# ChicyChen/LOCO-Edit

Measured on AMD Instinct MI355X. Metric: edit-directions/sec (top-5 PMP-Jacobian SVD @256^2) + vT cos-sim vs ref, higher is better.
Workload: dtype bf16x3 (split-bf16 MFMA operands, fp32 accumulate + fp32 storage); 1 GPU; CelebA-HQ DDPM 256x256 top-5 local basis (l_eye-sized mask, L=2400), t=0.6T, 12 power iterations, one GPU; multi_gpu_form=single, probes_total=5, probes_per_gpu=5, kept=5, n_iter=12, mask_L=2400, weights=synthetic seed 0, streams=2

## Files before the change

loco-edit_amd/csrc/conv_bf16.hip:

```cpp
#include "kernels.h"
#include <cstdio>
#include <cstdlib>

namespace loco {

enum : int { PR_BF16X3 = 0, PR_F16 = 1 };
template <int PR, int TAPS, int MODE> void launch_tile_b(const ConvArgs& a, hipStream_t st);
template <int PR, int MODE> void launch_kcat_b(const ConvArgs& a, hipStream_t st);
template <int PR, int MODE> void launch_pair_b(const ConvArgs& a, hipStream_t st);
void launch_conv_gemm(const ConvArgs& a, hipStream_t st);
template <int PR> void launch_poly_b(const ConvArgs& a, hipStream_t st);
template <int PR> void launch_poly_in_b(const ConvArgs& a, hipStream_t st);

template <int PR>
static void launch_lowp(const ConvArgs& a, int taps, hipStream_t st) {
#ifdef LOCO_DIAG
    if (a.cot_d && (taps != 1 || a.gemm || a.nsplit > 1 || a.Cin2 > 0 || (a.Cout % conv_bf16_tile_couts(a)) != 0 || a.st_kind == ST_TAN || a.st_kind == ST_COT)) {
        fprintf(stderr, "loco: ConvArgs::cot_d on a launch whose epilogue has no norm-cotangent term (taps %d, gemm %d, nsplit %d, Cout %d, st_kind %d)\n",
                taps, a.gemm, a.nsplit, a.Cout, a.st_kind);
        abort();
    }
#endif
    if constexpr (PR == PR_BF16X3) {
        if (taps == 1 && a.gemm) { launch_conv_gemm(a, st); return; }
    }
    if (taps == 9 && a.poly == 2) { launch_poly_in_b<PR>(a, st); return; }
    if (taps == 9 && a.poly) { launch_poly_b<PR>(a, st); return; }
    if (taps == 9 && a.Cin2 > 0) {
        if (a.mode == CM_GN_SILU) launch_kcat_b<PR, CM_GN_SILU>(a, st);
        else if (a.mode == CM_GN_GELU) launch_kcat_b<PR, CM_GN_GELU>(a, st);
        else launch_kcat_b<PR, CM_TAN_SILU>(a, st);
        return;
    }
    if constexpr (PR == PR_BF16X3) {
        if (taps == 9 && a.pair) {
            switch (a.mode) {
                case CM_NONE: launch_pair_b<PR, CM_NONE>(a, st); break;
                case CM_GN_SILU: launch_pair_b<PR, CM_GN_SILU>(a, st); break;
                case CM_TAN_SILU: launch_pair_b<PR, CM_TAN_SILU>(a, st); break;
                default: launch_pair_b<PR, CM_COT_SILU>(a, st); break;
            }
            return;
        }
    }
    if (taps == 9) {
        switch (a.mode) {
            case CM_NONE: launch_tile_b<PR, 9, CM_NONE>(a, st); break;
            case CM_GN_SILU: launch_tile_b<PR, 9, CM_GN_SILU>(a, st); break;
            case CM_GN_GELU: launch_tile_b<PR, 9, CM_GN_GELU>(a, st); break;
            case CM_TAN_SILU: launch_tile_b<PR, 9, CM_TAN_SILU>(a, st); break;
            case CM_COT_SILU: launch_tile_b<PR, 9, CM_COT_SILU>(a, st); break;
            default: launch_tile_b<PR, 9, CM_GN>(a, st); break;
        }
    } else {
        switch (a.mode) {
            case CM_NONE: launch_tile_b<PR, 1, CM_NONE>(a, st); break;
            default: launch_tile_b<PR, 1, CM_GN>(a, st); break;
        }
    }
}
void launch_conv_bf16x3(const ConvArgs& a, int taps, hipStream_t st) { launch_lowp<PR_BF16X3>(a, taps, st); }
void launch_conv_f16(const ConvArgs& a, int taps, hipStream_t st) { launch_lowp<PR_F16>(a, taps, st); }

}
```

loco-edit_amd/csrc/conv_plan.hip:

```cpp
#include "kernels.h"
#include <cstdio>
#include <cstdlib>

namespace loco {

constexpr int BKC = 16;
constexpr int BKF = 8;

static const int kMT[6] = {128, 128, 32, 64, 128, 128}, kNT[6] = {128, 64, 128, 64, 256, 256};

static int env_int(const char* name, int dflt) {
    const char* e = getenv(name);
    return e ? atoi(e) : dflt;
}
static int pick_tile(int Cout, int HW) {
    if (HW >= 128) return Cout > 32 ? 0 : 2;
    return Cout > 64 ? 1 : 3;
}

static int conv_pick_nsplit(int Cin, int Cout, int Hout, int Wout, int B) {
    const int t = pick_tile(Cout, Hout * Wout);
    long blocks = (long)((Hout * Wout) / kNT[t]) * ((Cout + kMT[t] - 1) / kMT[t]) * B;
    int nchunks = (Cin + BKF - 1) / BKF;
    if (blocks >= 384 || nchunks < 8) return 1;
    int want = (int)((512 + blocks - 1) / blocks);
    int maxs = nchunks / 4;
    if (want > maxs) want = maxs;
    if (want > 32) want = 32;
    return want < 1 ? 1 : want;
}

static int conv_bf16_pick_tile(int Cout, int HW, int B, int tile_override) {
    if (B <= 1 && HW <= 1024 && HW >= 64 && (Cout % 64) == 0) return 3;
    int t = pick_tile(Cout, HW);
    if (t == 0 && HW >= 256) {
        if (tile_override >= 0) return tile_override;
        return 5;
    }
    return t;
}

constexpr int kTile0MaxHW = 65536;

static int bf16_tile_of(const ConvArgs& a, int tile_override = -1) {
    int tile = conv_bf16_pick_tile(a.Cout, a.Hout * a.Wout, a.B, tile_override);
    if (tile == 4) tile = 5;
    if (tile == 5 && a.taps == 1 && !a.gemm && a.B >= 2 && a.Hout * a.Wout <= kTile0MaxHW) return 0;
    if (a.stride == 2 && tile == 5) tile = 0;
    return tile;
}
static int tile_for(const ConvArgs& a, int prec, int tile_override) {
    return prec ? bf16_tile_of(a, tile_override) : pick_tile(a.Cout, a.Hout * a.Wout);
}
static int conv_bf16_tile_pixels(const ConvArgs& a) { return a.poly == 1 ? 512 : a.gemm ? 256 : kNT[a.tile]; }
int conv_bf16_tile_couts(const ConvArgs& a) { return a.gemm ? 64 * a.gemm_tm : kMT[a.tile]; }

static bool conv_poly_ok(const ConvEnv& e, const ConvArgs& a, int taps) {
    static const bool on = env_int("LOCO_POLYPHASE", 1) != 0;
    if (!on || e.prec < 1 || taps != 9 || a.mode != CM_NONE || !(a.upsample || a.zins) || a.stride != 1) return false;
    if (!(e.prec == 2 ? a.wph : a.wpb) || !a.in_padded || a.res || a.Cin2 > 0 || a.cot_d) return false;
    if (a.upsample ? a.pad != 1 : (a.pad != 1 && a.pad != 2)) return false;
    if ((a.Cin % BKC) != 0 || (a.Cout % 128) != 0 || a.B < 2) return false;
    if (a.Hin * a.Win < 4096 || a.Win < 32 || (a.Win % 32) != 0 || (a.Hin % 8) != 0) return false;
    return a.Hout == 2 * a.Hin && a.Wout == 2 * a.Win;
}
static bool conv_poly_in_ok(const ConvEnv& e, const ConvArgs& a, int taps) {
    static const bool on = env_int("LOCO_POLYPHASE", 1) != 0;
    if (!on || e.prec < 1 || taps != 9 || a.mode != CM_NONE || !a.pool2 || a.upsample || a.zins || a.stride != 1 || a.pad != 1) return false;
    if (!(e.prec == 2 ? a.wqh : a.wqb) || a.res || a.bias2 || a.Cin2 > 0 || a.cot_d) return false;
    if ((a.Cin % BKC) != 0 || (a.Cout % 128) != 0 || a.B < 2 || ((a.Hin | a.Win) & 1)) return false;
    if (a.Hout * a.Wout < 4096 || a.Wout < 32 || (a.Wout % 32) != 0 || (a.Hout % 8) != 0) return false;
    return a.Hin == 2 * a.Hout && a.Win == 2 * a.Wout;
}

static int conv_bf16_pick_nsplit(int Cin, int Cout, int Hout, int Wout, int B, int chip_share, int taps, int lanes) {
    const int HW = Hout * Wout;
    int t = conv_bf16_pick_tile(Cout, HW, B, -1);
    if (t == 4) t = 5;
    if (taps == 1 && t == 5 && B >= 2 && HW <= kTile0MaxHW) t = 0;
    long blocks = (long)(HW / kNT[t]) * ((Cout + kMT[t] - 1) / kMT[t]) * B;
    int nchunks = (Cin + BKC - 1) / BKC;
    int target = chip_share > 1 ? 256 / chip_share : (lanes == 2 ? 240 : 256);
    if (target < 32) target = 32;
    if (blocks >= target / 2 || nchunks < 8) return 1;
    int want = (int)(target / blocks);
    int maxs = nchunks / 4;
    if (want > maxs) want = maxs;
    if (want > 32) want = 32;
    return want < 1 ? 1 : want;
}

static bool conv_lowp_can_kcat(const ConvArgs& a) {
    static const bool on = env_int("LOCO_KCAT", 1) != 0;
    return on && a.Cin2 > 0 && a.nsplit == 1 && bf16_tile_of(a) == 5 && a.stride == 1 && !a.upsample && !a.zins && a.pad == 1 &&
           (a.Cin % BKC) == 0 && (a.Cin2 % BKC) == 0 && a.in_padded &&
           (a.mode == CM_GN_SILU || a.mode == CM_GN_GELU || a.mode == CM_TAN_SILU);
}
static bool conv_lowp_can_fuse_stats(const ConvArgs& a) {
    return a.nsplit <= 1 && !a.gemm && (a.Cout % conv_bf16_tile_couts(a)) == 0;
}

static bool conv_pair_ok(const ConvArgs& a) {
    static const bool on = env_int("LOCO_CONV_PAIR", 1) != 0;
    if (!on || a.poly || a.Hout * a.Wout < 16384 || a.taps != 9 || a.Cin2 > 0 || a.nsplit != 1 || a.stride != 1 || a.upsample || a.zins ||
        a.pad != 1 || !a.in_padded || (a.Cin % (2 * BKC)) != 0 || (a.Cout % 128) != 0 || (a.Wout % 32) != 0 || (a.Hout % 8) != 0)
        return false;
    if (!(a.mode == CM_NONE || a.mode == CM_GN_SILU || a.mode == CM_TAN_SILU || a.mode == CM_COT_SILU)) return false;
    return a.tile == 5;
}

static ConvArgs conv_shift_batch(const ConvArgs& a, int nb) {
    ConvArgs t = a;
    t.B = a.B - nb;
    t.in += (long)nb * a.in_bs; t.out += (long)nb * a.out_bs;
    if (t.prim) t.prim += (long)nb * a.prim_bs;
    if (t.bias2) t.bias2 += (long)nb * a.bias2_bs;
    if (t.res) t.res += (long)nb * a.res_bs;
    if (t.sc) { t.sc += (long)nb * a.scsh_bs; t.sh += (long)nb * a.scsh_bs; }
    if (t.mr) t.mr += (long)nb * a.mr_bs;
    if (t.tst) t.tst += (long)nb * a.tst_bs;
    if (t.tc) t.tc += (long)nb * a.tc_bs;
    if (t.in2) t.in2 += (long)nb * a.in2_bs;
    if (t.cot_d) { t.cot_d += (long)nb * a.cot_d_bs; t.cot_tc += (long)nb * a.cot_tc_bs; }
    if (t.st_part) t.st_part += (long)nb * a.Cout * ((a.Hout * a.Wout) / conv_bf16_tile_pixels(a)) * 2;
    return t;
}

static void conv_gemm_plan(ConvArgs& a) {
    static const bool on = env_int("LOCO_CONV_GEMM", 1) != 0;
    a.gemm = 0;
    const long HW = (long)a.Hout * a.Wout;
    if (!on || a.stride != 1 || a.upsample || a.zins || (a.Cin % BKC) != 0 || a.Cin < 320 || (HW % 256) != 0 || (a.Wout % 16) != 0 ||
        a.Cout < 128 || !a.partial || a.Cin2 > 0 || !(a.mode == CM_NONE || a.mode == CM_GN) || a.cot_d)
        return;
    {
        const int TW = a.Wout < 32 ? a.Wout : 32;
        if ((256 % TW) != 0 || (a.Wout % TW) != 0 || (a.Hout % (256 / TW)) != 0) return;
    }
    static const int all_shapes = env_int("LOCO_GEMM_ALL", 0);
    if (!all_shapes && !(a.Cout >= 640 && (a.Cout >= 4 * a.Cin || a.Cin >= 2560))) return;
    const int pad256 = (a.Cout + 255) / 256 * 256;
    const int tm = (pad256 * 10 <= a.Cout * 11) ? 4 : 2;
    const int mt = 64 * tm;
    const long tiles = (HW / 256) * ((a.Cout + mt - 1) / mt) * a.B;
    const size_t rec_floats = (size_t)a.B * a.Cin * HW;
    int ns = 1;
    if (tiles < 192) {
        const int nchunks = a.Cin / BKC;
        ns = (int)((256 + tiles - 1) / tiles);
        if (ns > 8) ns = 8;
        while (ns > 1 && nchunks / ns < 8) --ns;
        while (ns > 1 && (size_t)ns * a.B * a.Cout * HW + rec_floats > a.partial_floats) --ns;
    }
    if ((ns > 1 ? (size_t)ns * a.B * a.Cout * HW : 0) + rec_floats > a.partial_floats) return;
    a.gemm = 1; a.gemm_tm = tm; a.nsplit = ns;
}

void conv_plan_family(ConvArgs& a, int prec) {
    if (prec == 1 && a.taps == 1) conv_gemm_plan(a);
}

// ... 16 lines not shown
    const int nchunks = (a.Cin + 15) / 16;
    while (s > 1 && nchunks / s < 4) --s;
    const size_t one = (size_t)(r / per_probe) * a.Cout * a.Hout * a.Wout;
    while (s > 1 && (size_t)s * one > partial_floats) --s;
    *split = s;
    return s > 1 ? (int)(r / per_probe) : 0;
}

static int stats_route(const ConvEnv& e, const StatAsk* q, bool want, ConvArgs& x, int s0, int B, int* keep_ntile) {
    if (!q || q->kind == ST_NONE) return SR_NONE;
    const int alone = q->norm ? SR_ALONE : SR_NONE;
    if (!want) return alone;
    if (x.nsplit > 1) return !q->norm ? SR_NONE : ((x.Hout * x.Wout) % 4 == 0 ? SR_SPLITK : SR_ALONE);
    const int ntile = (x.Hout * x.Wout) / conv_bf16_tile_pixels(x);
    const size_t need = (size_t)x.B * x.Cout * ntile * 2;
    const int epi = q->norm ? SR_EPI : SR_KEEP;
    const bool kept = q->keep && s0 == 0 && x.B == B && need <= q->keep_floats;
    if (q->kind == ST_FWD && x.poly != 1 && conv_lowp_can_fuse_stats(x) && (kept || (q->norm && need <= e.stpart_floats))) {
        x.st_part = kept ? q->keep : e.stpart; x.st_kind = ST_FWD;
        if (kept) *keep_ntile = ntile;
        return epi;
    }
    const bool cot_cache = q->kind == ST_COT && q->norm && q->sx && x.poly != 1;
    if ((q->kind == ST_TAN || cot_cache) && e.fuse_lin && !x.cot_d && conv_lowp_can_fuse_stats(x)) {
        const size_t lane_off = (size_t)e.lane_s0 * (q->keep_floats / e.max_batch);
        const bool keptl = q->kind == ST_TAN && q->keep && s0 == 0 && x.B == B && lane_off + need <= q->keep_floats;
        if (keptl || (q->norm && need <= e.stpart_floats)) {
            x.st_part = keptl ? q->keep + lane_off : e.stpart; x.st_kind = q->kind; x.st_x = q->prim;
            if (q->kind == ST_COT) x.st_sx = q->sx;
            if (keptl) *keep_ntile = ntile;
            return epi;
        }
    }
    return alone;
}

static ConvLaunch plan_launch(const ConvEnv& e, const StatAsk* q, bool want, const ConvArgs& x, int s0, int B, int* keep_ntile) {
    ConvLaunch l;
    l.args = x;
    l.s0 = s0;
    l.args.tile = tile_for(x, e.prec, -1);
    l.stats = stats_route(e, q, want, l.args, s0, B, keep_ntile);
    if (l.stats == SR_EPI || l.stats == SR_KEEP) l.ntile = (x.Hout * x.Wout) / conv_bf16_tile_pixels(l.args);
    conv_plan_tile_pair(l.args, e.prec, -1);
    return l;
}

ConvPlan plan_conv(const ConvEnv& e, const ConvArgs& a0, int taps, const StatAsk* q, const ConvArgs* sc) {
    ConvPlan p;
    ConvArgs a = a0;
    a.taps = taps;
    a.gemm = 0;
    a.poly = 0;
    if (a.pool2) {
        if (conv_poly_in_ok(e, a, taps)) a.poly = 2;
        else {
            p.pool_after = true; p.pool_out = a.out; p.pool_out_bs = a.out_bs; p.pool_acc = a.accumulate;
            a.out = a.pool_tmp; a.out_bs = a.pool_tmp_bs; a.Hout = a.Hin; a.Wout = a.Win; a.accumulate = 0; a.pool2 = 0;
        }
    }
    if (sc) {
        ConvArgs t = a;
        t.nsplit = e.prec >= 1 ? conv_bf16_pick_nsplit(a.Cin, a.Cout, a.Hout, a.Wout, a.B, e.chip_share, 9, e.lanes) : 2;
        t.in2 = sc->in; t.in2_bs = sc->in_bs; t.Cin2 = sc->Cin;
        const long per_probe = (long)((a.Hout * a.Wout) / 256) * ((a.Cout + 127) / 128);
        if (e.prec >= 1 && taps == 9 && !short_tail(per_probe, a.B) && !a.bias2 && conv_lowp_can_kcat(t)) {
            a.in2 = sc->in; a.in2_bs = sc->in_bs; a.Cin2 = sc->Cin; a.in2_padded = sc->in_padded;
            a.wb2 = e.prec == 2 ? sc->wh : sc->wb;
            a.bias2 = sc->bias; a.bias2_bs = 0;
            a.res = nullptr;
        } else {
            p.sc_first = true;
            a.res = sc->out; a.res_bs = sc->out_bs;
        }
    }
    if (e.prec == 2) a.wb = a.wh;
    a.no_deep = e.deep1 ? 0 : 1;
    a.nsplit = e.prec >= 1 ? conv_bf16_pick_nsplit(a.Cin, a.Cout, a.Hout, a.Wout, a.B, e.chip_share, taps, e.lanes)
                           : conv_pick_nsplit(a.Cin, a.Cout, a.Hout, a.Wout, a.B);
    if (a.cot_d) {
        ConvArgs t = a;
        t.tile = bf16_tile_of(t);
        const long per_probe = (long)((a.Hout * a.Wout) / conv_bf16_tile_pixels(t)) * ((a.Cout + 127) / 128);
        p.cot = e.prec >= 1 && taps == 1 && a.nsplit == 1 && !short_tail(per_probe, a.B) && conv_lowp_can_fuse_stats(t);
        if (!p.cot) { a.cot_d = nullptr; a.cot_d_bs = 0; a.cot_sx = nullptr; a.cot_tc = nullptr; a.cot_tc_bs = 0; }
    }
    while (a.nsplit > 1 && (size_t)a.nsplit * a.B * a.Cout * a.Hout * a.Wout > e.partial_floats) a.nsplit >>= 1;
    if (a.nsplit < 1) a.nsplit = 1;
    a.partial = e.partial;
    a.partial_floats = e.partial_floats;
    if (!a.poly && conv_poly_ok(e, a, taps)) a.poly = 1;
    if (a.poly == 1) { a.nsplit = 1; a.wb = e.prec == 2 ? a.wph : a.wpb; }
    if (a.poly == 2) { a.nsplit = 1; a.wb = e.prec == 2 ? a.wqh : a.wqb; }
    conv_plan_family(a, e.prec);
    a.tile = tile_for(a, e.prec, -1);
    int split = 1;
    const int tail = e.prec >= 1 && a.nsplit == 1 && a.B >= 2 && !a.gemm && !a.poly ? tail_split(a, e.partial_floats, &split) : 0;
    const bool want = q && q->kind != ST_NONE && e.prec >= 1 && e.fuse_stats;
    if (!tail) {
        p.l[0] = plan_launch(e, q, want, a, 0, a.B, &p.keep_ntile);
        return p;
    }
    const bool per_part = want && q->norm && (q->kind == ST_FWD || (e.fuse_lin && (a.Hout * a.Wout) % 4 == 0));
    p.stats_all = !per_part && q && q->kind != ST_NONE && q->norm;
    const StatAsk* ql = per_part ? q : nullptr;
    const int nb = a.B - tail;
    ConvArgs m = a, t = conv_shift_batch(a, nb);
    m.B = nb;
    t.nsplit = split;
    p.nl = 2;
    p.l[0] = plan_launch(e, ql, want, m, 0, a.B, &p.keep_ntile);
    p.l[1] = plan_launch(e, ql, want, t, nb, a.B, &p.keep_ntile);
    return p;
}

void polyphase_fold(int kind, int nin, int nout, const float* w, long so, long si, long st, float* out) {
    static const int sel[3][2][2][3] = {
        {{{1, 0, 0}, {0, 1, 1}}, {{1, 1, 0}, {0, 0, 1}}},
        {{{1, 0, 0}, {0, 0, 1}}, {{0, 1, 0}, {0, 0, 0}}},
        {{{0, 0, 0}, {0, 1, 0}}, {{1, 0, 0}, {0, 0, 1}}}};
    const long V = 4L * nout;
    for (int i = 0; i < nin; ++i)
        for (int pa = 0; pa < 2; ++pa)
            for (int pb = 0; pb < 2; ++pb)
                for (int ty = 0; ty < 2; ++ty)
                    for (int tx = 0; tx < 2; ++tx)
                        for (int o = 0; o < nout; ++o) {
                            double acc = 0.0;
                            for (int ky = 0; ky < 3; ++ky)
                                for (int kx = 0; kx < 3; ++kx)
                                    if (sel[kind][pa][ty][ky] && sel[kind][pb][tx][kx]) acc += (double)w[o * so + i * si + (3 * ky + kx) * st];
                            out[((long)i * 4 + 2 * ty + tx) * V + polyphase_vcout(nout, pa, pb, o)] = (float)acc;
                        }
}

void polyphase_fold_in(int nin, int nout, const float* w, long so, long si, long st, float* out, int noutP) {
    for (int p = 0; p < 2; ++p)
        for (int q = 0; q < 2; ++q)
            for (int i = 0; i < nin; ++i)
                for (int ty = 0; ty < 2; ++ty)
                    for (int tx = 0; tx < 2; ++tx) {
                        const int m = 2 * ty + 1 - p, n = 2 * tx + 1 - q;
                        for (int o = 0; o < nout; ++o) {
                            double acc = 0.0;
                            for (int a = 0; a < 2; ++a)
                                for (int b = 0; b < 2; ++b) {
                                    const int ky = m - a, kx = n - b;
                                    if (ky >= 0 && ky < 3 && kx >= 0 && kx < 3) acc += (double)w[o * so + i * si + (3 * ky + kx) * st];
                                }
                            out[((((long)(2 * p + q) * nin + i) * 4) + 2 * ty + tx) * noutP + o] = (float)acc;
                        }
                    }
}

const char* conv_variant_name(const ConvArgs& a, int taps, int prec) {
    static const char* tiles[6] = {"2,2,2,2", "4,1,1,2", "1,4,1,1", "2,2,1,1", "2,2,2,4", "2,4,2,2"};
    static char names[3][2][6][6][56];
    static char others[3][3][6][40];
    const int mode = (a.mode < 0 || a.mode > 5) ? 2 : a.mode;
    const char* other = nullptr;
    int k = 0, v = mode;
    if (prec && taps == 9 && a.poly) {
        static const char* pn[2][3] = {{"", "conv_mfma_bf16x3<4,2,4,2,2,0>", "conv_mfma_f16<4,2,4,2,2,0>"},
                                       {"", "conv_mfma_bf16x3<4,2,4,2,2,0>+pool", "conv_mfma_f16<4,2,4,2,2,0>+pool"}};
        return pn[a.poly == 2][prec];
    }
    if (prec && taps == 9 && a.Cin2 > 0) other = prec == 1 ? "conv_kcat_bf16x3<2,4,2,2,%d>" : "conv_kcat_f16<2,4,2,2,%d>";
    else if (prec == 1 && taps == 1 && a.gemm) { k = 1; other = "conv_gemm_bf16x3<%d>"; v = a.gemm_tm; }
    else if (prec == 1 && taps == 9 && a.pair) { k = 2; other = "conv_pair_bf16x3<%d>"; }
    if (other) {
        char* n = others[k][prec][v];
        if (!n[0]) snprintf(n, 40, other, v);
        return n;
    }
    int t = a.tile;
    if (t < 0 || t > 5) t = 0;
    int m = mode;
    if (taps != 9 && m != CM_NONE) m = CM_GN;
    if (!prec && m == CM_GN_GELU) m = CM_GN_SILU;
    char* n = names[prec][taps == 9 ? 0 : 1][t][m];
    static const char* kn[3] = {"conv_mfma_f32", "conv_mfma_bf16x3", "conv_mfma_f16"};
    if (!n[0]) snprintf(n, 56, "%s<%d,%s,%d>", kn[prec], taps, tiles[t], m);
    return n;
}

}
```

loco-edit_amd/csrc/conv_plan_text.h:

```cpp
#pragma once
#include "kernels.h"
#include <cstdio>
#include <string>

namespace loco {

inline const char* stat_route_name(int r) {
    static const char* names[5] = {"none", "epi", "splitk", "alone", "keep"};
    return r >= 0 && r < 5 ? names[r] : "?";
}

inline void conv_plan_text(const ConvPlan& p, int taps, int prec, std::string& out) {
    char line[384];
    for (int li = 0; li < p.nl; ++li) {
        const ConvLaunch& l = p.l[li];
        const ConvArgs& y = l.args;
        snprintf(line, sizeof(line),
                 "launch=%d part=0 kernel=%s tile=%d nsplit=%d B=%d s0=%d gemm=%d gemm_tm=%d pair=%d Cin2=%d sc_first=%d cot=%d "
                 "stats=%s ntile=%d\n",
                 li, conv_variant_name(y, taps, prec), y.tile, y.nsplit, y.B, l.s0, y.gemm, y.gemm ? y.gemm_tm : 0, y.pair, y.Cin2,
                 p.sc_first ? 1 : 0, p.cot ? 1 : 0, stat_route_name(l.stats), l.ntile);
        out += line;
    }
    snprintf(line, sizeof(line), "stats_all=%d keep_ntile=%d\n", p.stats_all ? 1 : 0, p.keep_ntile);
    out += line;
}

}
```

loco-edit_amd/csrc/engine_internal.h:

```cpp
#pragma once
#include <hip/hip_runtime.h>

#include <cstdint>
#include <cstring>
#include <map>
#include <memory>
#include <string>
#include <vector>

#include "../../include/loco_hip.h"
#include "kernels.h"
#include "program.h"

#define HIPCHK(ctx, call)                                                                    \
    do {                                                                                     \
        hipError_t e_ = (call);                                                              \
        if (e_ != hipSuccess) {                                                              \
            (ctx)->err = std::string(#call) + ": " + hipGetErrorString(e_);                  \
            return -1;                                                                       \
        }                                                                                    \
    } while (0)

namespace loco {
namespace eng {

struct ConvP {
    float* wf = nullptr;
    float* wd = nullptr;
    float* wbf = nullptr;
    float* wbd = nullptr;
    float* whf = nullptr;
    float* whd = nullptr;
    float* wpb = nullptr;
    float* wph = nullptr;
    bool poly_dgrad = false;
    float* wqb = nullptr;
    float* wqh = nullptr;
    float* bias = nullptr;
    int cin = 0, cout = 0, taps = 0;
};
struct NormW { float* gamma = nullptr; float* beta = nullptr; };

struct OpWeights {
    ConvP c1, c2, nin, qkvc, proj, conv;
    ConvP xqc, xproj;
    ConvP pj_in, to_out1, to_out2, ff1, ff2, pj_out;
    NormW g1, g2, gx;
    float *xkw = nullptr, *xkb = nullptr, *xvw = nullptr, *xvb = nullptr;
    float *xng = nullptr, *xnb = nullptr;
    float *lng[3] = {nullptr, nullptr, nullptr}, *lnb[3] = {nullptr, nullptr, nullptr};
    long tproj_off = 0;
};
struct Weights {
    std::vector<OpWeights> op;
    float *freq = nullptr, *td0w = nullptr, *td0b = nullptr, *td1w = nullptr, *td1b = nullptr;
    float* tcw = nullptr;
    float *tp_w = nullptr, *tp_b = nullptr;
    long tproj_total = 0;
    double flops = 0.0;
};

struct Tens : TensPlan {
    float* keep = nullptr; size_t keep_floats = 0; int keep_ntile = 0;
};
struct NormP : NormPlan, NormW {
    bool ready = false;
};
struct Op : OpPlan, OpWeights {
    NormP n1, n2, nx;
    float *xK = nullptr, *xV = nullptr;
};

struct HostParam { std::vector<float> data; std::vector<int64_t> shape; bool loaded = false; };

}
}


struct loco_ctx {
    loco_unet_cfg cfg;
    std::string err;
    std::map<std::string, loco::eng::HostParam> params;
    bool finalized = false;

    std::shared_ptr<const loco::Program> prog;
    std::shared_ptr<loco::eng::Weights> wts;
    std::vector<loco::eng::Tens> tens;
    std::vector<loco::eng::Op> ops;


// ... 84 lines not shown
        return ev_pool[ev_used++];
    }
};

namespace loco {
namespace eng {

template <typename T>
int dalloc(loco_ctx* c, T** p, size_t count) {
    void* q = nullptr;
    HIPCHK(c, hipMalloc(&q, count * sizeof(T)));
    *p = reinterpret_cast<T*>(q);
    c->owned.push_back(reinterpret_cast<float*>(q));
    c->bytes += count * sizeof(T);
    return 0;
}

inline float eps_of(const loco_ctx* c, const NormP& n) { return n.eps > 0.f ? n.eps : c->cfg.gn_eps; }
int upload(loco_ctx* c, float** dst, const std::vector<float>& h);

int make_conv(loco_ctx* c, const std::vector<const HostParam*>& ws, const std::vector<const HostParam*>& bs,
              ConvP* out, int row_limit = -1, int poly_kind = -1, bool poly_dgrad = false);
int make_conv1(loco_ctx* c, const std::string& name, ConvP* out, int row_limit = -1, int poly_kind = -1, bool poly_dgrad = false);
int make_conv1_scaled(loco_ctx* c, const std::string& name, ConvP* out, float s);
int make_norm(loco_ctx* c, const std::string& name, NormW* n);
int bind_weights(loco_ctx* c);
int finalize_params(loco_ctx* c);

struct NS { float *sc, *sh, *mr, *tst, *tc; };
NS nstats(const loco_ctx* c, float* base, const NormP& n);

struct StatReq {
    int kind = ST_NONE;
    NormP* n = nullptr;
    float* stats = nullptr;
    const float* prim = nullptr;
    const float* ss_scale = nullptr; const float* ss_shift = nullptr;
    float* keep = nullptr; size_t keep_floats = 0; int* keep_ntile = nullptr;
};

inline void conv_defaults(ConvArgs& a) {
    std::memset(&a, 0, sizeof(a));
    a.stride = 1; a.pad = 1; a.nsplit = 1; a.mode = CM_NONE; a.res_scale = 1.f;
}
inline void setw(ConvArgs& a, const ConvP& p, bool dgrad) {
    a.w = dgrad ? p.wd : p.wf;
    a.wb = dgrad ? (const void*)p.wbd : (const void*)p.wbf;
    a.wh = dgrad ? (const void*)p.whd : (const void*)p.whf;
    const bool folded = p.wpb && p.poly_dgrad == dgrad;
    a.wpb = folded ? p.wpb : nullptr;
    a.wph = folded ? p.wph : nullptr;
    a.wqb = dgrad ? p.wqb : nullptr;
    a.wqh = dgrad ? p.wqh : nullptr;
}

struct TView {
    float* p; long bs; int C, H, W;
    operator float*() const { return p; }
};
inline TView tview(const loco_ctx* c, float* arena, int id) {
    const Tens& t = c->tens[id];
    return {arena + t.off, c->prog->per_sample, t.C, t.H, t.W};
}
inline TView tview_in(const float* p, long bs, int C, int H, int W) { return {const_cast<float*>(p), bs, C, H, W}; }
inline ConvArgs conv_args(const TView& in, const ConvP& w, bool dgrad, const TView& out, int B, int ksize) {
    ConvArgs a; conv_defaults(a);
    a.in = in.p; a.in_bs = in.bs; a.Cin = in.C; a.Hin = in.H; a.Win = in.W;
    setw(a, w, dgrad);
    a.out = out.p; a.out_bs = out.bs; a.Cout = out.C; a.Hout = out.H; a.Wout = out.W; a.B = B;
    if (ksize == 1) a.pad = 0;
    return a;
}
bool run_conv(loco_ctx* c, const ConvArgs& a0, int taps, hipStream_t st, const StatReq* rq = nullptr,
              const ConvArgs* second = nullptr);

struct XA {
    loco_ctx* c; hipStream_t st; int B; int C, T, NH, CH, L, Lp;
    float scale;
    const float *xK, *xV;
    const float* colbias;
    long xs, ss;
};
void xa_forward(const XA& x, const float* Xq, float* P, float* O);
void xa_linear(const XA& x, const float* X, const float* K1, const float* K2, float* P, float* S, float* O);
int xa_context_grad(const XA& x, const Op& op, const float* go, const float* q, const float* P, float* S);

struct Attn {
    loco_ctx* c; hipStream_t st;
    int B, T, NH, CH, Lt, Tk;
    long HS, SS, OS, KS;
    float scale;
    bool pair;
    const float *q, *k, *v, *P, *o;
    float *tq, *tk, *tv, *tS, *to;
    long bq, bS, bo;
    const float *kt, *vt;
    const float* colbias;
    float* delta;
    unsigned char* ws; size_t ws_bytes;
    bool flash() const {
        return c->flash_attn && c->prec >= 1 && (Lt ? attn_flash_text_supported(T, CH, Lt) : attn_flash_supported(T, CH));
    }
};
AttnFlashArgs attn_flash_args(const Attn& s);
void attn_forward(const Attn& s);
void attn_tangent(const Attn& s);
// ... 5 lines not shown
```

loco-edit_amd/csrc/engine_params.hip:

```cpp
#include <atomic>
#include <cmath>
#include <cstring>
#include <thread>

#include "engine_internal.h"

namespace loco {
namespace eng {

static inline uint16_t f2bf(float f) {
    uint32_t u; std::memcpy(&u, &f, 4);
    u += 0x7FFFu + ((u >> 16) & 1u);
    return (uint16_t)(u >> 16);
}
static inline float bf2f(uint16_t h) {
    uint32_t u = (uint32_t)h << 16; float f; std::memcpy(&f, &u, 4); return f;
}
template <typename F>
static void parallel_for(int n, size_t work, F fn) {
    unsigned nt = std::thread::hardware_concurrency();
    if (nt > 16) nt = 16;
    if ((int)nt > n) nt = (unsigned)n;
    if (nt <= 1 || work < ((size_t)1 << 18)) { for (int i = 0; i < n; ++i) fn(i); return; }
    std::atomic<int> next{0};
// ... 36 lines not shown
        for (int t = 0; t < taps; ++t)
            for (int o = 0; o < nout; ++o) {
                _Float16* r = rec.data() + (((size_t)ck * taps + t) * noutP + o) * 16;
                int sw = (o >> 3) & 1;
                for (int k = 0; k < 16; ++k) {
                    int i = ck * 16 + k;
                    float v = (i < nin) ? get(o, i, t) : 0.f;
                    r[((k >> 3) ^ sw) * 8 + (k & 7)] = (_Float16)v;
                }
            }
    });
    std::vector<float> out(rec.size() / 2);
    std::memcpy(out.data(), rec.data(), rec.size() * 2);
    return out;
}

int make_conv(loco_ctx* c, const std::vector<const HostParam*>& ws, const std::vector<const HostParam*>& bs,
              ConvP* out, int row_limit, int poly_kind, bool poly_dgrad) {
    int cin = (int)ws[0]->shape[1], k = ws[0]->shape.size() > 2 ? (int)ws[0]->shape[2] : 1;
    int taps = ws[0]->shape.size() == 4 ? k * k : k;
    int cout = 0;
    for (auto* w : ws) cout += (int)w->shape[0];
    if (row_limit > 0 && ws.size() == 1 && row_limit < cout) cout = row_limit;
    int coutP = (cout + 31) & ~31, cinP = (cin + 31) & ~31;
    std::vector<float> wf((size_t)cin * taps * coutP, 0.f), wd((size_t)cout * taps * cinP, 0.f), bias(cout);
    int co0 = 0;
    for (size_t wi = 0; wi < ws.size(); ++wi) {
        const HostParam* w = ws[wi];
        int co_n = (int)w->shape[0];
        if (co_n > cout - co0) co_n = cout - co0;
        parallel_for(co_n, (size_t)co_n * cin * taps, [&](int co) {
            for (int ci = 0; ci < cin; ++ci)
                for (int t = 0; t < taps; ++t)
                    wd[((size_t)(co0 + co) * taps + (taps - 1 - t)) * cinP + ci] = w->data[((size_t)co * cin + ci) * taps + t];
        });
        parallel_for(cin, (size_t)co_n * cin * taps, [&](int ci) {
            for (int t = 0; t < taps; ++t)
                for (int co = 0; co < co_n; ++co)
                    wf[((size_t)ci * taps + t) * coutP + co0 + co] = w->data[((size_t)co * cin + ci) * taps + t];
        });
        for (int co = 0; co < co_n; ++co) bias[co0 + co] = bs[wi]->data[co];
        co0 += co_n;
    }
    out->cin = cin; out->cout = cout; out->taps = taps;
    if (upload(c, &out->wf, wf) || upload(c, &out->wd, wd) || upload(c, &out->bias, bias)) return -1;
    auto fwd = [&](int o, int i, int t) { return wf[((size_t)i * taps + t) * coutP + o]; };
    auto dgr = [&](int o, int i, int t) { return wd[((size_t)i * taps + t) * cinP + o]; };
    std::vector<float> rf = build_records(cin, cout, taps, fwd);
    std::vector<float> rd = build_records(cout, cin, taps, dgr);
    if (upload(c, &out->wbf, rf) || upload(c, &out->wbd, rd)) return -1;
    std::vector<float> hf = build_records_f16(cin, cout, taps, fwd);
    std::vector<float> hd = build_records_f16(cout, cin, taps, dgr);
    if (upload(c, &out->whf, hf) || upload(c, &out->whd, hd)) return -1;
    const int pin = poly_dgrad ? cout : cin, pout = poly_dgrad ? cin : cout;
    if (poly_kind >= 0 && taps == 9 && pin % 16 == 0 && pout % 128 == 0) {
        const int poutP = poly_dgrad ? cinP : coutP;
        std::vector<float> pf((size_t)pin * 16 * pout);
        polyphase_fold(poly_kind, pin, pout, (poly_dgrad ? wd : wf).data(), 1, 9L * poutP, poutP, pf.data());
        auto fold = [&](int o, int i, int t) { return pf[((size_t)i * 4 + t) * 4 * pout + o]; };
        std::vector<float> rp = build_records(pin, 4 * pout, 4, fold), hp = build_records_f16(pin, 4 * pout, 4, fold);
        if (upload(c, &out->wpb, rp) || upload(c, &out->wph, hp)) return -1;
        out->poly_dgrad = poly_dgrad;
    }
    if (poly_kind == POLY_UP && !poly_dgrad && taps == 9 && cout % 16 == 0 && cin % 128 == 0) {
        std::vector<float> qf((size_t)4 * cout * 4 * cinP, 0.f);
        polyphase_fold_in(cout, cin, wd.data(), 1, 9L * cinP, cinP, qf.data(), cinP);
        auto fold = [&](int o, int i, int t) { return qf[((size_t)i * 4 + t) * cinP + o]; };
        std::vector<float> rq = build_records(4 * cout, cin, 4, fold), hq = build_records_f16(4 * cout, cin, 4, fold);
        if (upload(c, &out->wqb, rq) || upload(c, &out->wqh, hq)) return -1;
    }
    return 0;
}
int make_conv1(loco_ctx* c, const std::string& name, ConvP* out, int row_limit, int poly_kind, bool poly_dgrad) {
    return make_conv(c, {&c->params[name + ".weight"]}, {&c->params[name + ".bias"]}, out, row_limit, poly_kind, poly_dgrad);
}
int make_conv1_scaled(loco_ctx* c, const std::string& name, ConvP* out, float s) {
    if (s == 1.f) return make_conv1(c, name, out);
    HostParam w = c->params[name + ".weight"], b = c->params[name + ".bias"];
    for (float& v : w.data) v *= s;
    for (float& v : b.data) v *= s;
    return make_conv(c, {&w}, {&b}, out);
}
int make_norm(loco_ctx* c, const std::string& name, NormW* n) {
    if (upload(c, &n->gamma, c->params[name + ".weight"].data)) return -1;
    if (upload(c, &n->beta, c->params[name + ".bias"].data)) return -1;
    return 0;
}

int bind_weights(loco_ctx* c) {
    const Weights& W = *c->wts;
    for (size_t i = 0; i < c->ops.size(); ++i) {
        Op& v = c->ops[i];
        static_cast<OpWeights&>(v) = W.op[i];
        static_cast<NormW&>(v.n1) = v.g1; static_cast<NormW&>(v.n2) = v.g2; static_cast<NormW&>(v.nx) = v.gx;
    }
    if (dalloc(c, &c->tact, (size_t)c->cfg.ch * 4) || dalloc(c, &c->tproj, (size_t)(W.tproj_total > 0 ? W.tproj_total : 1))) return -1;
    c->finalized = true;
    return 0;
}

int finalize_params(loco_ctx* c) {
    if (c->finalized) return 0;
    for (const ParamDecl& d : c->prog->params)
        if (!c->params[d.name].loaded) { c->err = "parameter not loaded: " + d.name; return -1; }
    Weights& W = *c->wts;
    const loco_unet_cfg& cfg = c->cfg;
// ... 154 lines not shown
```

loco-edit_amd/csrc/kernels.h:

```cpp
#pragma once
#include <hip/hip_runtime.h>
#include <stdint.h>

namespace loco {

struct DeviceOnce { bool seen[64] = {}; };
inline bool first_on_device(DeviceOnce& f) {
    int d = 0;
    (void)hipGetDevice(&d);
    d &= 63;
    if (f.seen[d]) return false;
    f.seen[d] = true;
    return true;
}


enum ConvMode : int {
    CM_NONE = 0,
    CM_GN_SILU = 1,
    CM_GN = 2,
    CM_TAN_SILU = 3,
    CM_COT_SILU = 4,
    CM_GN_GELU = 5,
};
// ... 3 lines not shown
    return y * (1.0f / (1.0f + __expf(-y)));
}
__device__ __forceinline__ float act_der(float y, int act) {
    if (act == ACT_GELU) return 0.5f * (1.0f + erff(y * 0.70710678118654752f)) + y * 0.39894228040143268f * __expf(-0.5f * y * y);
    const float sg = 1.0f / (1.0f + __expf(-y));
    return sg * (1.0f + y * (1.0f - sg));
}

enum StatKind : int { ST_NONE = 0, ST_FWD = 1, ST_TAN = 2, ST_COT = 3 };

struct ConvArgs {
    const float* in; long in_bs; int Cin, Hin, Win;
    const float* prim; long prim_bs;
    const float* w;
    const void* wb;
    const void* wh;
    const float2* sx;
    float* out; long out_bs; int Cout, Hout, Wout;
    const float* bias;
    const float* bias2; long bias2_bs;
    const float* res; long res_bs;
    const float* sc; const float* sh; long scsh_bs;
    const float* mr; long mr_bs;
    const float* gamma_;
    const float* tst; long tst_bs;
    const float* tc; long tc_bs;
    int cpg;
    int mode;
    int stride;
    int pad;
    int upsample;
    int zins;
    int in_padded;
    int accumulate;
    int nsplit;
    int taps;
    int no_deep;
    float* partial;
    int B;
    float* st_part; int st_kind;
    const float* st_x; const float2* st_sx;
    const float* in2; long in2_bs; int Cin2; int in2_padded;
    const void* wb2;
    const float* cot_d; long cot_d_bs; const float2* cot_sx; const float* cot_tc; long cot_tc_bs;
    int act;
    float res_scale;
    int gemm, gemm_tm;
    size_t partial_floats;
    int tile, pair;
    const void* wpb; const void* wph;
    int poly;
    int pool2; float* pool_tmp; long pool_tmp_bs;
    const void* wqb; const void* wqh;
};

enum PolyKind : int { POLY_UP = 0, POLY_ZINS_PAD2 = 1, POLY_ZINS_PAD1 = 2 };
inline int polyphase_vcout(int C, int a, int b, int co) { return ((a * (C / 64) + co / 64) * 2 + b) * 64 + (co % 64); }
void polyphase_fold(int kind, int nin, int nout, const float* w, long so, long si, long st, float* out);
void polyphase_fold_in(int nin, int nout, const float* w, long so, long si, long st, float* out, int noutP);

void launch_conv(const ConvArgs& a, int taps, hipStream_t st);
void launch_conv_bf16x3(const ConvArgs& a, int taps, hipStream_t st);
void launch_conv_f16(const ConvArgs& a, int taps, hipStream_t st);
void launch_conv_splitk_reduce(const ConvArgs& a, hipStream_t st);

struct ConvEnv {
    int prec = 1;
    int chip_share = 1;
    int lanes = 1, lane_s0 = 0;
    float* partial = nullptr; size_t partial_floats = 0;
    float* stpart = nullptr; size_t stpart_floats = 0;
    bool fuse_stats = true, fuse_lin = true, deep1 = true;
    int max_batch = 1;
};

struct StatAsk {
    int kind = ST_NONE;
    bool norm = false;
    const float2* sx = nullptr;
    const float* prim = nullptr;
    float* keep = nullptr; size_t keep_floats = 0;
};

enum StatRoute : int {
    SR_NONE = 0,
    SR_EPI = 1,
    SR_SPLITK = 2,
    SR_ALONE = 3,
    SR_KEEP = 4,
};

struct ConvLaunch {
    ConvArgs args;
    int s0 = 0;
    int stats = SR_NONE;
    int ntile = 0;
};

struct ConvPlan {
    bool sc_first = false;
    int nl = 1;
    ConvLaunch l[2];
    bool stats_all = false;
    int keep_ntile = 0;
    bool pool_after = false; float* pool_out = nullptr; long pool_out_bs = 0; int pool_acc = 0;
    bool cot = false;
};
// ... 215 lines not shown
```

Before: 20.56 edit-directions/s.

## Add specialised 3x3 conv kernels for thin-channel UNet input/output ends

Adds two bf16x3 MFMA kernels for the UNet's end convolutions. The first covers a tiny Cin (9*Cin<=32) with many output channels: it folds all taps into a single K=32 slice, keeps the weights in registers and reads an input halo from LDS. The second covers a tiny Cout (9*Cout<=32): it computes the per-tap partial products as an M=27 GEMM over input channels, then sums the shifted taps from LDS in a scalar epilogue. The general tiled kernels waste most of their MFMA tile and K-chunk work on these shapes, and that waste is what this removes. In exchange the change adds new weight packings, planner routing and an env switch, and the new epilogues skip the stats and split-K paths.

```diff
diff --git a/loco-edit_amd/csrc/conv_bf16.hip b/loco-edit_amd/csrc/conv_bf16.hip
--- a/loco-edit_amd/csrc/conv_bf16.hip
+++ b/loco-edit_amd/csrc/conv_bf16.hip
@@ -11,6 +11,8 @@
 void launch_conv_gemm(const ConvArgs& a, hipStream_t st);
 template <int PR> void launch_poly_b(const ConvArgs& a, hipStream_t st);
 template <int PR> void launch_poly_in_b(const ConvArgs& a, hipStream_t st);
+void launch_ends_k(const ConvArgs& a, hipStream_t st);
+void launch_ends_m(const ConvArgs& a, hipStream_t st);
 
 template <int PR>
 static void launch_lowp(const ConvArgs& a, int taps, hipStream_t st) {
@@ -23,6 +25,10 @@
 #endif
     if constexpr (PR == PR_BF16X3) {
         if (taps == 1 && a.gemm) { launch_conv_gemm(a, st); return; }
+    }
+    if constexpr (PR == PR_BF16X3) {
+        if (taps == 9 && a.ends == 1) { launch_ends_k(a, st); return; }
+        if (taps == 9 && a.ends == 2) { launch_ends_m(a, st); return; }
     }
     if (taps == 9 && a.poly == 2) { launch_poly_in_b<PR>(a, st); return; }
     if (taps == 9 && a.poly) { launch_poly_b<PR>(a, st); return; }
diff --git a/loco-edit_amd/csrc/conv_bf16_inst_m.hip b/loco-edit_amd/csrc/conv_bf16_inst_m.hip
--- /dev/null
+++ b/loco-edit_amd/csrc/conv_bf16_inst_m.hip
@@ -0,0 +1,5 @@
+#include "conv_ends_kernel.h"
+
+namespace loco {
+void launch_ends_m(const ConvArgs& a, hipStream_t st) { launch_ends_m_impl(a, st); }
+}
diff --git a/loco-edit_amd/csrc/conv_bf16_inst_n.hip b/loco-edit_amd/csrc/conv_bf16_inst_n.hip
--- /dev/null
+++ b/loco-edit_amd/csrc/conv_bf16_inst_n.hip
@@ -0,0 +1,5 @@
+#include "conv_ends_kernel.h"
+
+namespace loco {
+void launch_ends_k(const ConvArgs& a, hipStream_t st) { launch_ends_k_impl(a, st); }
+}
diff --git a/loco-edit_amd/csrc/conv_ends_kernel.h b/loco-edit_amd/csrc/conv_ends_kernel.h
--- /dev/null
+++ b/loco-edit_amd/csrc/conv_ends_kernel.h
@@ -0,0 +1,198 @@
+#pragma once
+#include "conv_bf16_kernel.h"
+
+namespace loco {
+
+constexpr int ENDS_TH = 8, ENDS_TW = 32;
+constexpr int ENDS_HW = ENDS_TW + 2, ENDS_HH = ENDS_TH + 2;
+constexpr int ENDS_HALO = ENDS_HW * ENDS_HH;
+
+template <int PR>
+__global__ __launch_bounds__(512) void conv_ends_k_bf16x3(ConvArgs a) {
+    static_assert(PR == PR_BF16X3, "split-bf16 records");
+    constexpr int WM = 2, WN = 4, TM = 2, TN = 2, MT = 128, NT = 256;
+    extern __shared__ __attribute__((aligned(16))) unsigned char smem_b[];
+    float* const H = reinterpret_cast<float*>(smem_b);
+    const int tid = threadIdx.x, lane = tid & 63, wave = tid >> 6;
+    const int l31 = lane & 31, khalf = lane >> 5, wm = wave / WN, wn = wave % WN;
+    const int ncot = a.Cout / MT, tiles_x = a.Wout / ENDS_TW;
+    int L = blockIdx.x;
+    const int b = L % a.B; L /= a.B;
+    const int cot_id = L % ncot, tile_id = L / ncot;
+    const int oy0 = (tile_id / tiles_x) * ENDS_TH, ox0 = (tile_id % tiles_x) * ENDS_TW;
+    const int co0 = cot_id * MT;
+
+    s16x8 ah[TM][2], al[TM][2];
+    {
+        const uint4* wk = reinterpret_cast<const uint4*>(a.wb);
+#pragma unroll
+        for (int i = 0; i < TM; ++i) {
+            const uint4* r = wk + (long)(co0 + (wm * TM + i) * 32 + l31) * 8;
+#pragma unroll
+            for (int s = 0; s < 2; ++s) {
+                ah[i][s] = __builtin_bit_cast(s16x8, r[s * 4 + khalf]);
+                al[i][s] = __builtin_bit_cast(s16x8, r[s * 4 + 2 + khalf]);
+            }
+        }
+    }
+    {
+        const float* inb = a.in + (long)b * a.in_bs;
+        const int n = a.Cin * ENDS_HALO, plane = a.Hin * a.Win;
+        for (int e = tid; e < n; e += 512) {
+            const int ci = e / ENDS_HALO, r = e - ci * ENDS_HALO;
+            const int hy = r / ENDS_HW, hx = r - hy * ENDS_HW;
+            const int iy = oy0 + hy - 1, ix = ox0 + hx - 1;
+            float v = 0.f;
+            if (iy >= 0 && iy < a.Hin && ix >= 0 && ix < a.Win) v = inb[(long)ci * plane + iy * a.Win + ix];
+            H[e] = v;
+        }
+    }
+    int koff[2][8];
+    unsigned kmask = 0;
+#pragma unroll
+    for (int s = 0; s < 2; ++s)
+#pragma unroll
+        for (int i = 0; i < 8; ++i) {
+            const int k = 16 * s + 8 * khalf + i;
+            const bool live = k < 9 * a.Cin;
+            const int t = live ? idiv_small(k, a.Cin) : 0, ci = live ? k - t * a.Cin : 0;
+            const int ky = (t * 11) >> 5, kx = t - 3 * ky;
+            koff[s][i] = ci * ENDS_HALO + ky * ENDS_HW + kx;
+            kmask |= (live ? 1u : 0u) << (s * 8 + i);
+        }
+    __syncthreads();
+    f32x16 acc[TM][TN];
+#pragma unroll
+    for (int i = 0; i < TM; ++i)
+#pragma unroll
+        for (int j = 0; j < TN; ++j)
+#pragma unroll
+            for (int r = 0; r < 16; ++r) acc[i][j][r] = 0.f;
+#pragma unroll
+    for (int j = 0; j < TN; ++j) {
+        const int p = (wn * TN + j) * 32 + l31;
+        const int pix = (p >> 5) * ENDS_HW + (p & 31);
+#pragma unroll
+        for (int s = 0; s < 2; ++s) {
+            float x[8];
+#pragma unroll
+            for (int i = 0; i < 8; ++i) {
+                const float v = H[koff[s][i] + pix];
+                x[i] = ((kmask >> (s * 8 + i)) & 1u) ? v : 0.f;
+            }
+            uint4 h4, l4;
+            split8<PR_BF16X3>(x, h4, l4);
+            const bf16x8 bh = __builtin_bit_cast(bf16x8, h4), bl = __builtin_bit_cast(bf16x8, l4);
+#pragma unroll
+            for (int i = 0; i < TM; ++i) {
+                const bf16x8 wh = __builtin_bit_cast(bf16x8, ah[i][s]), wl = __builtin_bit_cast(bf16x8, al[i][s]);
+                acc[i][j] = __builtin_amdgcn_mfma_f32_32x32x16_bf16(wl, bh, acc[i][j], 0, 0, 0);
+                acc[i][j] = __builtin_amdgcn_mfma_f32_32x32x16_bf16(wh, bl, acc[i][j], 0, 0, 0);
+                acc[i][j] = __builtin_amdgcn_mfma_f32_32x32x16_bf16(wh, bh, acc[i][j], 0, 0, 0);
+            }
+        }
+    }
+    __syncthreads();
+    conv_lowp_epilogue<WM, WN, TM, TN, EPI_STATS>(a, acc, smem_b, co0, oy0, ox0, ENDS_TW, tile_id, b, 0);
+}
+
+inline void launch_ends_k_impl(const ConvArgs& a, hipStream_t st) {
+    const size_t lds = (size_t)2 * 32 * 256 * 4;
+    dim3 grid((unsigned)(((a.Hout * a.Wout) / 256) * (a.Cout / 128) * a.B));
+    hipLaunchKernelGGL(conv_ends_k_bf16x3<PR_BF16X3>, grid, dim3(512), lds, st, a);
+}
+
+constexpr int ENDS_NBLK = (ENDS_HALO + 31) / 32;
+constexpr int ENDS_YP = ENDS_NBLK * 32;
+
+template <int PR>
+__global__ __launch_bounds__(256) void conv_ends_m_bf16x3(ConvArgs a) {
+    static_assert(PR == PR_BF16X3, "split-bf16 records");
+    constexpr int NB = 3;
+    __shared__ float Ys[27 * ENDS_YP];
+    const int tid = threadIdx.x, lane = tid & 63, wave = tid >> 6;
+    const int l31 = lane & 31, khalf = lane >> 5;
+    const int tiles_x = a.Wout / ENDS_TW;
+    const int b = blockIdx.x % a.B, tile_id = blockIdx.x / a.B;
+    const int oy0 = (tile_id / tiles_x) * ENDS_TH, ox0 = (tile_id % tiles_x) * ENDS_TW;
+    const int plane = a.Hin * a.Win, nch = a.Cin / BKC;
+
+    unsigned poff[NB];
+    bool pin[NB];
+#pragma unroll
+    for (int n = 0; n < NB; ++n) {
+        const int q = (wave + 4 * n) * 32 + l31;
+        const int hy = q / ENDS_HW, hx = q - hy * ENDS_HW;
+        const int iy = oy0 + hy - 1, ix = ox0 + hx - 1;
+        pin[n] = q < ENDS_HALO && iy >= 0 && iy < a.Hin && ix >= 0 && ix < a.Win;
+        poff[n] = pin[n] ? (unsigned)(iy * a.Win + ix) : 0u;
+    }
+    const bool last = wave + 4 * (NB - 1) < ENDS_NBLK;
+    const float* inb = a.in + (long)b * a.in_bs;
+    const uint4* wm = reinterpret_cast<const uint4*>(a.wb);
+
+    f32x16 acc[NB];
+#pragma unroll
+    for (int n = 0; n < NB; ++n)
+#pragma unroll
+        for (int r = 0; r < 16; ++r) acc[n][r] = 0.f;
+
+    for (int ck = 0; ck < nch; ++ck) {
+        const int c0 = ck * BKC + 8 * khalf;
+        const uint4* wr = wm + ((long)ck * 32 + l31) * 4;
+        const bf16x8 wh = __builtin_bit_cast(bf16x8, wr[khalf]), wl = __builtin_bit_cast(bf16x8, wr[2 + khalf]);
+        const float* ip = inb + (long)c0 * plane;
+#pragma unroll
+        for (int n = 0; n < NB; ++n) {
+            if (n == NB - 1 && !last) break;
+            float d[8], x[8];
+#pragma unroll
+            for (int i = 0; i < 8; ++i) d[i] = ip[(unsigned)i * (unsigned)plane + poff[n]];
+#pragma unroll
+            for (int i = 0; i < 8; ++i) x[i] = pin[n] ? d[i] : 0.f;
+            uint4 h4, l4;
+            split8<PR_BF16X3>(x, h4, l4);
+            const bf16x8 bh = __builtin_bit_cast(bf16x8, h4), bl = __builtin_bit_cast(bf16x8, l4);
+            acc[n] = __builtin_amdgcn_mfma_f32_32x32x16_bf16(wl, bh, acc[n], 0, 0, 0);
+            acc[n] = __builtin_amdgcn_mfma_f32_32x32x16_bf16(wh, bl, acc[n], 0, 0, 0);
+            acc[n] = __builtin_amdgcn_mfma_f32_32x32x16_bf16(wh, bh, acc[n], 0, 0, 0);
+        }
+    }
+#pragma unroll
+    for (int n = 0; n < NB; ++n) {
+        if (n == NB - 1 && !last) break;
+        const int q = (wave + 4 * n) * 32 + l31;
+#pragma unroll
+        for (int r = 0; r < 16; ++r) {
+            const int row = (r & 3) + 8 * (r >> 2) + 4 * khalf;
+            if (row < 27) Ys[row * ENDS_YP + q] = acc[n][r];
+        }
+    }
+    __syncthreads();
+    {
+        const int ty = tid >> 5, tx = tid & 31;
+        const long out_plane = (long)a.Hout * a.Wout;
+        const long o = (long)(oy0 + ty) * a.Wout + ox0 + tx;
+        float* const ob = a.out + (long)b * a.out_bs;
+        const float* const rb = a.res ? a.res + (long)b * a.res_bs : nullptr;
+        const float* const b2 = a.bias2 ? a.bias2 + (long)b * a.bias2_bs : nullptr;
+        const float* yp = Ys + ty * ENDS_HW + tx;
+        for (int co = 0; co < a.Cout; ++co) {
+            float v = 0.f;
+#pragma unroll
+            for (int t = 0; t < 9; ++t) v += yp[(co * 9 + t) * ENDS_YP + (t / 3) * ENDS_HW + (t % 3)];
+            if (a.bias) v += a.bias[co];
+            if (b2) v += b2[co];
+            if (rb) v = fmaf(a.res_scale, rb[co * out_plane + o], v);
+            if (a.accumulate) v += ob[co * out_plane + o];
+            ob[co * out_plane + o] = v;
+        }
+    }
+}
+
+inline void launch_ends_m_impl(const ConvArgs& a, hipStream_t st) {
+    dim3 grid((unsigned)(((a.Hout * a.Wout) / 256) * a.B));
+    hipLaunchKernelGGL(conv_ends_m_bf16x3<PR_BF16X3>, grid, dim3(256), 0, st, a);
+}
+
+}
diff --git a/loco-edit_amd/csrc/conv_plan.hip b/loco-edit_amd/csrc/conv_plan.hip
--- a/loco-edit_amd/csrc/conv_plan.hip
+++ b/loco-edit_amd/csrc/conv_plan.hip
@@ -1,6 +1,7 @@
 #include "kernels.h"
 #include <cstdio>
 #include <cstdlib>
+#include <cstring>
 
 namespace loco {
 
@@ -102,11 +103,28 @@
 
 static bool conv_pair_ok(const ConvArgs& a) {
     static const bool on = env_int("LOCO_CONV_PAIR", 1) != 0;
-    if (!on || a.poly || a.Hout * a.Wout < 16384 || a.taps != 9 || a.Cin2 > 0 || a.nsplit != 1 || a.stride != 1 || a.upsample || a.zins ||
+    if (!on || a.poly || a.ends || a.Hout * a.Wout < 16384 || a.taps != 9 || a.Cin2 > 0 || a.nsplit != 1 || a.stride != 1 || a.upsample || a.zins ||
         a.pad != 1 || !a.in_padded || (a.Cin % (2 * BKC)) != 0 || (a.Cout % 128) != 0 || (a.Wout % 32) != 0 || (a.Hout % 8) != 0)
         return false;
     if (!(a.mode == CM_NONE || a.mode == CM_GN_SILU || a.mode == CM_TAN_SILU || a.mode == CM_COT_SILU)) return false;
     return a.tile == 5;
+}
+
+static bool conv_ends_common(const ConvEnv& e, const ConvArgs& a, int taps, int form) {
+    static const int sw = env_int("LOCO_CONV_ENDS", 1);
+    const bool on = sw == 1 || sw == 1 + form;
+    if (!on || e.prec != 1 || taps != 9 || a.stride != 1 || a.pad != 1 || a.upsample || a.zins || a.pool2 || a.poly) return false;
+    if (a.Cin2 > 0 || a.cot_d || a.Hin != a.Hout || a.Win != a.Wout) return false;
+    return a.Hout * a.Wout >= 4096 && (a.Wout % 32) == 0 && (a.Hout % 8) == 0;
+}
+static bool conv_ends_k_ok(const ConvEnv& e, const ConvArgs& a, int taps) {
+    return conv_ends_common(e, a, taps, 1) && a.wkb && a.mode == CM_NONE && 9 * a.Cin <= 32 && (a.Cout % 128) == 0 && a.nsplit == 1;
+}
+static bool conv_ends_m_ok(const ConvEnv& e, const ConvArgs& a, int taps, const StatAsk* q) {
+    if (!conv_ends_common(e, a, taps, 2) || !a.wmb || !a.in_padded || (a.Cin % BKC) != 0 || 9 * a.Cout > 32) return false;
+    if (q && q->kind != ST_NONE) return false;
+    if (a.nsplit > 1 && a.Cin > 8 * BKC) return false;
+    return a.mode == CM_NONE;
 }
 
 static ConvArgs conv_shift_batch(const ConvArgs& a, int nb) {
@@ -229,6 +247,7 @@
     a.taps = taps;
     a.gemm = 0;
     a.poly = 0;
+    a.ends = 0;
     if (a.pool2) {
         if (conv_poly_in_ok(e, a, taps)) a.poly = 2;
         else {
@@ -269,10 +288,13 @@
     if (!a.poly && conv_poly_ok(e, a, taps)) a.poly = 1;
     if (a.poly == 1) { a.nsplit = 1; a.wb = e.prec == 2 ? a.wph : a.wpb; }
     if (a.poly == 2) { a.nsplit = 1; a.wb = e.prec == 2 ? a.wqh : a.wqb; }
+    if (!sc && conv_ends_k_ok(e, a, taps)) a.ends = 1;
+    else if (!sc && conv_ends_m_ok(e, a, taps, q)) a.ends = 2;
+    if (a.ends) { a.nsplit = 1; a.wb = a.ends == 1 ? a.wkb : a.wmb; }
     conv_plan_family(a, e.prec);
     a.tile = tile_for(a, e.prec, -1);
     int split = 1;
-    const int tail = e.prec >= 1 && a.nsplit == 1 && a.B >= 2 && !a.gemm && !a.poly ? tail_split(a, e.partial_floats, &split) : 0;
+    const int tail = e.prec >= 1 && a.nsplit == 1 && a.B >= 2 && !a.gemm && !a.poly && !a.ends ? tail_split(a, e.partial_floats, &split) : 0;
     const bool want = q && q->kind != ST_NONE && e.prec >= 1 && e.fuse_stats;
     if (!tail) {
         p.l[0] = plan_launch(e, q, want, a, 0, a.B, &p.keep_ntile);
@@ -330,6 +352,40 @@
                     }
 }
 
+static inline uint16_t ends_bf16(float f) {
+    uint32_t u;
+    memcpy(&u, &f, 4);
+    u += 0x7FFFu + ((u >> 16) & 1u);
+    return (uint16_t)(u >> 16);
+}
+static inline void ends_split(float v, uint16_t* hi, uint16_t* lo) {
+    *hi = ends_bf16(v);
+    const uint32_t u = (uint32_t)*hi << 16;
+    float h;
+    memcpy(&h, &u, 4);
+    *lo = ends_bf16(v - h);
+}
+void conv_ends_pack_k(int nin, int nout, const float* w, long so, long si, long st, uint16_t* out) {
+    for (int o = 0; o < nout; ++o)
+        for (int k = 0; k < 32; ++k) {
+            const int t = k / nin, i = k - t * nin;
+            const float v = k < 9 * nin ? w[o * so + i * si + t * st] : 0.f;
+            uint16_t* r = out + (size_t)o * 64 + (k >> 4) * 32 + (k & 15);
+            ends_split(v, r, r + 16);
+        }
+}
+void conv_ends_pack_m(int nin, int nout, const float* w, long so, long si, long st, uint16_t* out) {
+    for (int ck = 0; ck < nin / 16; ++ck)
+        for (int r = 0; r < 32; ++r) {
+            const int o = r / 9, t = r - 9 * o;
+            for (int k = 0; k < 16; ++k) {
+                const float v = r < 9 * nout ? w[o * so + (ck * 16 + k) * si + t * st] : 0.f;
+                uint16_t* p = out + ((size_t)ck * 32 + r) * 32 + k;
+                ends_split(v, p, p + 16);
+            }
+        }
+}
+
 const char* conv_variant_name(const ConvArgs& a, int taps, int prec) {
     static const char* tiles[6] = {"2,2,2,2", "4,1,1,2", "1,4,1,1", "2,2,1,1", "2,2,2,4", "2,4,2,2"};
     static char names[3][2][6][6][56];
@@ -342,6 +398,8 @@
                                        {"", "conv_mfma_bf16x3<4,2,4,2,2,0>+pool", "conv_mfma_f16<4,2,4,2,2,0>+pool"}};
         return pn[a.poly == 2][prec];
     }
+    if (prec == 1 && taps == 9 && a.ends == 1) return "conv_ends_k_bf16x3<0>";
+    if (prec == 1 && taps == 9 && a.ends == 2) return "conv_ends_m_bf16x3<0>";
     if (prec && taps == 9 && a.Cin2 > 0) other = prec == 1 ? "conv_kcat_bf16x3<2,4,2,2,%d>" : "conv_kcat_f16<2,4,2,2,%d>";
     else if (prec == 1 && taps == 1 && a.gemm) { k = 1; other = "conv_gemm_bf16x3<%d>"; v = a.gemm_tm; }
     else if (prec == 1 && taps == 9 && a.pair) { k = 2; other = "conv_pair_bf16x3<%d>"; }
diff --git a/loco-edit_amd/csrc/conv_plan_text.h b/loco-edit_amd/csrc/conv_plan_text.h
--- a/loco-edit_amd/csrc/conv_plan_text.h
+++ b/loco-edit_amd/csrc/conv_plan_text.h
@@ -21,6 +21,11 @@
                  li, conv_variant_name(y, taps, prec), y.tile, y.nsplit, y.B, l.s0, y.gemm, y.gemm ? y.gemm_tm : 0, y.pair, y.Cin2,
                  p.sc_first ? 1 : 0, p.cot ? 1 : 0, stat_route_name(l.stats), l.ntile);
         out += line;
+        if (y.ends) {
+            out.pop_back();
+            snprintf(line, sizeof(line), " ends=%d\n", y.ends);
+            out += line;
+        }
     }
     snprintf(line, sizeof(line), "stats_all=%d keep_ntile=%d\n", p.stats_all ? 1 : 0, p.keep_ntile);
     out += line;
diff --git a/loco-edit_amd/csrc/engine_internal.h b/loco-edit_amd/csrc/engine_internal.h
--- a/loco-edit_amd/csrc/engine_internal.h
+++ b/loco-edit_amd/csrc/engine_internal.h
@@ -36,6 +36,8 @@
     bool poly_dgrad = false;
     float* wqb = nullptr;
     float* wqh = nullptr;
+    float *wkf = nullptr, *wkd = nullptr;
+    float *wmf = nullptr, *wmd = nullptr;
     float* bias = nullptr;
     int cin = 0, cout = 0, taps = 0;
 };
@@ -226,6 +228,8 @@
     a.wph = folded ? p.wph : nullptr;
     a.wqb = dgrad ? p.wqb : nullptr;
     a.wqh = dgrad ? p.wqh : nullptr;
+    a.wkb = dgrad ? p.wkd : p.wkf;
+    a.wmb = dgrad ? p.wmd : p.wmf;
 }
 
 struct TView {
diff --git a/loco-edit_amd/csrc/engine_params.hip b/loco-edit_amd/csrc/engine_params.hip
--- a/loco-edit_amd/csrc/engine_params.hip
+++ b/loco-edit_amd/csrc/engine_params.hip
@@ -112,6 +112,22 @@
     std::vector<float> hf = build_records_f16(cin, cout, taps, fwd);
     std::vector<float> hd = build_records_f16(cout, cin, taps, dgr);
     if (upload(c, &out->whf, hf) || upload(c, &out->whd, hd)) return -1;
+    if (taps == 9) {
+        auto ends = [&](int nin, int nout, const std::vector<float>& w3, int noutP, float** wk, float** wm) -> int {
+            if (9 * nin <= 32 && nout % 128 == 0) {
+                std::vector<float> r((size_t)nout * 32);
+                conv_ends_pack_k(nin, nout, w3.data(), 1, 9L * noutP, noutP, reinterpret_cast<uint16_t*>(r.data()));
+                if (upload(c, wk, r)) return -1;
+            }
+            if (9 * nout <= 32 && nin % 16 == 0) {
+                std::vector<float> r((size_t)(nin / 16) * 32 * 16);
+                conv_ends_pack_m(nin, nout, w3.data(), 1, 9L * noutP, noutP, reinterpret_cast<uint16_t*>(r.data()));
+                if (upload(c, wm, r)) return -1;
+            }
+            return 0;
+        };
+        if (ends(cin, cout, wf, coutP, &out->wkf, &out->wmf) || ends(cout, cin, wd, cinP, &out->wkd, &out->wmd)) return -1;
+    }
     const int pin = poly_dgrad ? cout : cin, pout = poly_dgrad ? cin : cout;
     if (poly_kind >= 0 && taps == 9 && pin % 16 == 0 && pout % 128 == 0) {
         const int poutP = poly_dgrad ? cinP : coutP;
diff --git a/loco-edit_amd/csrc/kernels.h b/loco-edit_amd/csrc/kernels.h
--- a/loco-edit_amd/csrc/kernels.h
+++ b/loco-edit_amd/csrc/kernels.h
@@ -79,7 +79,12 @@
     int poly;
     int pool2; float* pool_tmp; long pool_tmp_bs;
     const void* wqb; const void* wqh;
-};
+    const void* wkb; const void* wmb;
+    int ends;
+};
+
+void conv_ends_pack_k(int nin, int nout, const float* w, long so, long si, long st, uint16_t* out);
+void conv_ends_pack_m(int nin, int nout, const float* w, long so, long si, long st, uint16_t* out);
 
 enum PolyKind : int { POLY_UP = 0, POLY_ZINS_PAD2 = 1, POLY_ZINS_PAD1 = 2 };
 inline int polyphase_vcout(int C, int a, int b, int co) { return ((a * (C / 64) + co / 64) * 2 + b) * 64 + (co % 64); }
```

Result: no change. 20.61 edit-directions/s (median of 6 runs) (+0.2%).
